# SharperJBCA/COMAPreduce

Measured on AMD Instinct MI355X. Metric: TOD samples x channels / s (L1 -> L2 reduction), higher is better.
Workload: dtype f32 in, f64 accumulate

## Files before the change

comapreduce_amd/csrc/l1_kernels.hip:

```cpp
#include "comap_internal.h"

#include <algorithm>
#include <cfloat>
#include <cmath>
#include <cstdlib>
#include <cstring>
#include <type_traits>
#include <utility>

using namespace comap;

#ifndef COMAP_GROUPS
#define COMAP_GROUPS 0
#endif
constexpr int kGroupsAutoMin = 3;

typedef float f32x4u __attribute__((ext_vector_type(4), aligned(4)));
__device__ __forceinline__ f32x4u ld4(const float *p)
{
    return __builtin_nontemporal_load(reinterpret_cast<const f32x4u *>(p));
}

__device__ __forceinline__ double wave_sum(double v)
{
// ... 911 lines not shown
                __double_as_longlong(kap[UC + i]) != __double_as_longlong(krfa) ||
                __double_as_longlong(kap[2 * UC + i]) != __double_as_longlong(kofa))
                atomicOr(flag, 1);
        }
        kap[i] = kgfa;
        kap[UC + i] = krfa;
        kap[2 * UC + i] = kofa;
        s_kap[0][c] = al;
        s_kap[1][c] = kgfa;
        s_kap[2][c] = krfa;
        s_kap[3][c] = kofa;
        if (fused) {
            const double sd = mom[i] - n * o - a * SA;
            if (kgfa != 0.0) { acc[0] += kgfa * o; acc[1] += kgfa * a; acc[2] += kgfa * sd; }
            if (krfa != 0.0) { acc[3] += krfa * o; acc[4] += krfa * a; acc[5] += krfa * sd; }
            if (kofa != 0.0) { acc[6] += kofa * o; acc[7] += kofa * a; acc[8] += kofa * sd; }
            if (kr != 0.0) acc[9] += kr;
        } else {
            if (kg != 0.0) { acc[0] += kg * fb; acc[1] += kg * fg; acc[2] += kg * fd; }
            if (kr != 0.0) { acc[3] += kr * fb; acc[4] += kr * fg; acc[5] += kr * fd; acc[9] += kr; }
            if (ko != 0.0) { acc[6] += ko * fb; acc[7] += ko * fg; acc[8] += ko * fd; }
        }
        acc[10] += W;
        acc[11] += Wo;
    }
#pragma unroll
    for (int k = 0; k < 12; ++k) acc[k] = block_sum256(acc[k], red);
    if (threadIdx.x == 0 && phase != 0) {
        if (fused) {
            const double *P = pd + 4 * (int64_t)ub;
#pragma unroll
            for (int j = 0; j < 3; ++j) {
                const double sko = acc[3 * j], ska = acc[3 * j + 1], ksy = acc[3 * j + 2];
                const double ksym = P[j] - Smf * sko - SAm * ska;
                const double kx0 = (Smm * ksy - Smf * ksym) / det;
                const double kx1 = (n * ksym - Smf * ksy) / det;
                acc[3 * j] = -(sko + kx0);
                acc[3 * j + 1] = -ska;
                acc[3 * j + 2] = -kx1;
            }
        }
        double *o = dsum + 16 * (int64_t)ub;
#pragma unroll
        for (int k = 0; k < 12; ++k) o[k] = acc[k];
    }
    if (phase == 0) {
        pbad = block_sum256(pbad, red);
        pmag = block_sum256(pmag, red);
        if (threadIdx.x == 0) {
            pg[2 * (int64_t)ub] = pbad;
            pg[2 * (int64_t)ub + 1] = pmag + 1.0;
        }
    }
    __syncthreads();
    if (phase == 0 && threadIdx.x < 64) {
        double *w = dw + 4 * (int64_t)ub * kChannels;
        const int nc = wave_compact_channels(
            threadIdx.x, [&](int c) { return s_kap[0][c] != 0.0; },
            [&](int j, int c) {
#pragma unroll
                for (int k = 0; k < 4; ++k) w[4 * j + k] = s_kap[k][c];
            },
            [&](int j) {
#pragma unroll
                for (int k = 0; k < 4; ++k) w[4 * j + k] = 0.0;
            },
            dlist + (int64_t)ub * kChannels);
        if (threadIdx.x == 0) dcnt[ub] = nc;
    }
}

__global__ void __launch_bounds__(256) k_special_rows(int mode, const int32_t *__restrict__ units,
                                                      const float *__restrict__ tod, int64_t T,
                                                      const double *__restrict__ A, const double *__restrict__ mf,
                                                      const double *__restrict__ oa, const double *__restrict__ alpha,
                                                      const double *__restrict__ nf, const int32_t *__restrict__ rowbad,
                                                      const double *__restrict__ bsum, const double *__restrict__ xreg,
                                                      const double *__restrict__ tsys0, const double *__restrict__ gain0,
                                                      const double *__restrict__ dsum, int calibrator,
                                                      int32_t *__restrict__ ugate, double *__restrict__ tod_out,
                                                      double *__restrict__ orig_out)
{
    __shared__ int nrow;
    __shared__ int16_t rows[kChannels];
    __shared__ double rw[kChannels], rwo[kChannels];
    const int ub = blockIdx.x;
    const int u = ub / kBands, b = ub % kBands;
    if (mode == 0 && b != 0) return;
    const int f = units[4 * u], t0 = units[4 * u + 2], n = units[4 * u + 3];
    const bool band_on = bsum[4 * (int64_t)ub + 3] > 0;
    if (!band_on) return;
    const bool zero = mode == 1 && !calibrator && n >= 5 && !ugate[u];
    if (threadIdx.x == 0) nrow = 0;
    __syncthreads();
    const int64_t kb = (int64_t)u * kBC + b * kChannels, fb = (int64_t)f * kBC + b * kChannels;
    for (int c = threadIdx.x; c < kChannels; c += blockDim.x) {
        const int64_t i = kb + c;
        if (!special_row(band_on, c, alpha[i], rowbad[i])) continue;
        const double tsv = tsys0[fb + c];
        if (zero && (gain_masked(c) || isnan(tsv))) continue;
        const float d0 = tod[(fb + c) * T + t0];
        const double y0 = special_y(alpha[i], oa[2 * i], oa[2 * i + 1], xreg[2 * i], xreg[2 * i + 1], d0,
                                    A[(int64_t)f * T + t0], mf[((int64_t)f * kBands + b) * T + t0]);
        double W, Wo;
        special_weights(c, tsv, nf[i], gain0[fb + c], y0, W, Wo);
        const int k = atomicAdd(&nrow, 1);
        rows[k] = (int16_t)c;
        rw[k] = W;
        rwo[k] = Wo;
    }
    __syncthreads();
    const int nr = nrow;
    if (nr == 0) return;
    const double *a = A + (int64_t)f * T + t0;
    const double *m = mf + ((int64_t)f * kBands + b) * T + t0;
    if (mode == 0) {
        bool inf = false;
        for (int t = threadIdx.x; t < n; t += blockDim.x)
            for (int k = 0; k < nr; ++k) {
                const int64_t i = kb + rows[k];
                const double y = special_y(alpha[i], oa[2 * i], oa[2 * i + 1], xreg[2 * i], xreg[2 * i + 1],
                                           tod[(fb + rows[k]) * T + t0 + t], a[t], m[t]);
                inf |= isinf(y);
            }
        if (inf) ugate[u] = 1;
        return;
    }
    const double *ds = dsum + 16 * (int64_t)ub;
    const double SW = ds[10], SWo = ds[11];
    double *to = tod_out + ((int64_t)f * kBands + b) * T + t0;
    double *oo = orig_out + ((int64_t)f * kBands + b) * T + t0;
    for (int t = threadIdx.x; t < n; t += blockDim.x) {
        double sr = 0.0, so = 0.0;
        for (int k = 0; k < nr; ++k) {
            const int c = rows[k];
            const int64_t i = kb + c;
            const double y = special_y(alpha[i], oa[2 * i], oa[2 * i + 1], xreg[2 * i], xreg[2 * i + 1],
                                       tod[(fb + c) * T + t0 + t], a[t], m[t]);
            double r = y * nf[i] / gain0[fb + c];
            if (isnan(r)) r = 0.0;
            sr += rw[k] * r;
            double q = y * tsys0[fb + c];
            if (isnan(q)) q = 0.0;
            so += rwo[k] * q;
        }
        to[t] += sr / SW;
        oo[t] += so / SWo;
    }
}

__global__ void __launch_bounds__(256) k_gain_avg(const float *__restrict__ tod, const double *__restrict__ A,
                                                  const int32_t *__restrict__ units, const int32_t *__restrict__ tiles,
                                                  int64_t tile0, int64_t T, int64_t UC, const double *__restrict__ kap,
                                                  const double *__restrict__ dsum, const double *__restrict__ mf,
                                                  double *__restrict__ tod_out, double *__restrict__ orig_out,
                                                  double *__restrict__ dG_out, const int32_t *__restrict__ flag)
{
    __shared__ double sg[kBands][kTile];
    if (*flag == 0) return;
    const int b = uniform(threadIdx.x >> 6);
    const int lane = threadIdx.x & 63;
    const int64_t tile = tile0 + blockIdx.x;
    const int u = tiles[2 * tile], toff = tiles[2 * tile + 1];
    const int f = units[4 * u], t0 = units[4 * u + 2], n = units[4 * u + 3];
    const int r0 = toff + 4 * lane;
    const float *base = tod + (int64_t)(f * kBands + b) * kChannels * T + t0 + r0;
    const int64_t kb = (int64_t)u * kBC + b * kChannels;
    const double *kg = kap + kb, *kr = kap + UC + kb, *ko = kap + 2 * UC + kb;
    double ag[4 * kJ], ar[4 * kJ], ao[4 * kJ];
#pragma unroll
    for (int i = 0; i < 4 * kJ; ++i) ag[i] = ar[i] = ao[i] = 0.0;
    const int nv0 = n - r0;
#pragma unroll 2
    for (int c = 0; c < kChannels; ++c) {
        const double wg = kg[c], wr = kr[c], wo = ko[c];
        if (wg == 0.0 && wr == 0.0 && wo == 0.0) continue;
        double x[4 * kJ];
        load_groups(base + (int64_t)c * T, nv0, x);
#pragma unroll
        for (int i = 0; i < 4 * kJ; ++i) {
            ag[i] = fma(wg, x[i], ag[i]);
            ar[i] = fma(wr, x[i], ar[i]);
            ao[i] = fma(wo, x[i], ao[i]);
        }
    }
    const double *ds = dsum + 16 * ((int64_t)u * kBands + b);
    const double *a = A + (int64_t)f * T + t0 + r0;
    const double *m = mf + (int64_t)(f * kBands + b) * T + t0 + r0;
    double at[4 * kJ], mt[4 * kJ];
#pragma unroll
    for (int g = 0; g < kJ; ++g)
#pragma unroll
        for (int e = 0; e < 4; ++e) {
            const int i = 4 * g + e, o = 256 * g + e;
            const bool ok = o < nv0;
            at[i] = ok ? a[o] : 0.0;
            mt[i] = ok ? m[o] : 0.0;
            sg[b][256 * g + 4 * lane + e] = ag[i] + ds[0] + at[i] * ds[1] + mt[i] * ds[2];
        }
    __syncthreads();
    double *to = tod_out + (int64_t)(f * kBands + b) * T + t0 + r0;
    double *oo = orig_out + (int64_t)(f * kBands + b) * T + t0 + r0;
#pragma unroll
    for (int g = 0; g < kJ; ++g)
#pragma unroll
        for (int e = 0; e < 4; ++e) {
            const int i = 4 * g + e, o = 256 * g + e;
            if (o >= nv0) continue;
            const int tl = 256 * g + 4 * lane + e;
            const double dG = sg[0][tl] + sg[1][tl] + sg[2][tl] + sg[3][tl];
            const double sr = ar[i] + ds[3] + at[i] * ds[4] + mt[i] * ds[5];
            const double so = ao[i] + ds[6] + at[i] * ds[7] + mt[i] * ds[8];
            to[o] = (sr - dG * ds[9]) / ds[10];
            oo[o] = so / ds[11];
            if (b == 0) dG_out[(int64_t)f * T + t0 + r0 + o] = dG;
        }
}

__device__ __forceinline__ void scan_weight_band(const double *__restrict__ r, int n, double *__restrict__ wo,
                                                 double *red)
{
    const int np = n / 2;
    double s = 0, cnt = 0;
    for (int k = threadIdx.x; k < np; k += blockDim.x) {
        const double d = r[2 * k + 1] - r[2 * k];
        if (!isnan(d)) { s += d; cnt += 1.0; }
    }
    s = block_sum256(s, red);
    cnt = block_sum256(cnt, red);
    const double mean = s / cnt;
    double v = 0;
    for (int k = threadIdx.x; k < np; k += blockDim.x) {
        const double d = r[2 * k + 1] - r[2 * k];
        if (!isnan(d)) v += (d - mean) * (d - mean);
    }
    v = block_sum256(v, red);
    const double rms = sqrt(v / cnt) / sqrt(2.0);
    const double wt = 1.0 / (rms * rms);
    for (int t = threadIdx.x; t < n; t += blockDim.x) wo[t] = wt;
}

__global__ void __launch_bounds__(256) k_scan_weights(int ub0, const int32_t *__restrict__ units, int64_t T,
                                                      const double *__restrict__ tod_out, double *__restrict__ w_out)
{
    __shared__ double red[4];
    const int ub = ub0 + blockIdx.x;
    const int u = ub / kBands, b = ub % kBands;
    const int f = units[4 * u], t0 = units[4 * u + 2], n = units[4 * u + 3];
    const int64_t o = (int64_t)(f * kBands + b) * T + t0;
    scan_weight_band(tod_out + o, n, w_out + o, red);
}

__global__ void __launch_bounds__(256) k_finish(const int32_t *__restrict__ units, const int32_t *__restrict__ tiles,
                                                int64_t tile0, int64_t T, const double *__restrict__ A,
                                                const double *__restrict__ mf, const double *__restrict__ dsum,
                                                double *__restrict__ tod_out, double *__restrict__ orig_out,
                                                double *__restrict__ dG, const int32_t *__restrict__ flag)
{
    if (*flag != 0) return;
    const int64_t tile = tile0 + blockIdx.x;
    const int u = tiles[2 * tile];
    const int f = units[4 * u], t0 = units[4 * u + 2], n = units[4 * u + 3];
    const double *ds = dsum + 16 * (int64_t)u * kBands;
    for (int k = threadIdx.x; k < kTile; k += 256) {
        const int r = tiles[2 * tile + 1] + k;
        if (r >= n) break;
        const int64_t t = t0 + r;
        const double a = A[(int64_t)f * T + t];
        double m[kBands], g = dG[(int64_t)f * T + t];
#pragma unroll
        for (int b = 0; b < kBands; ++b) {
            m[b] = mf[(int64_t)(f * kBands + b) * T + t];
            const double *d = ds + 16 * b;
            g += d[0] + a * d[1] + m[b] * d[2];
        }
        dG[(int64_t)f * T + t] = g;
#pragma unroll
        for (int b = 0; b < kBands; ++b) {
            const double *d = ds + 16 * b;
            const int64_t o = (int64_t)(f * kBands + b) * T + t;
            tod_out[o] = (tod_out[o] + d[3] + a * d[4] + m[b] * d[5] - g * d[9]) / d[10];
            orig_out[o] = (orig_out[o] + d[6] + a * d[7] + m[b] * d[8]) / d[11];
        }
    }
}

__global__ void __launch_bounds__(256) k_zero_gaps(const int64_t *__restrict__ gaps, int64_t T, int F,
                                                   double *__restrict__ tod_out, double *__restrict__ orig_out,
                                                   double *__restrict__ w_out)
{
    const int64_t *g = gaps + 3 * (int64_t)blockIdx.y;
    const int64_t f = g[0], t0 = g[1], n = g[2];
    for (int64_t k = blockIdx.x * (int64_t)blockDim.x + threadIdx.x; k < n; k += (int64_t)gridDim.x * blockDim.x) {
#pragma unroll
        for (int b = 0; b < kBands; ++b) {
            const int64_t o = (f * kBands + b) * T + t0 + k;
            tod_out[o] = 0.0;
            orig_out[o] = 0.0;
            w_out[o] = 0.0;
        }
    }
}

__global__ void __launch_bounds__(256) k_vane(const float *__restrict__ tod, int64_t T, int F,
                                              int64_t vstart, const int32_t *__restrict__ hot,
                                              const int64_t *__restrict__ hoff, const int32_t *__restrict__ cold,
                                              const int64_t *__restrict__ coff, double t_hot,
                                              double *__restrict__ tsys, double *__restrict__ gain)
{
    __shared__ float s_cold[128];
    const int side = threadIdx.x >> 7;
    const int64_t row = (int64_t)blockIdx.x * 128 + (threadIdx.x & 127);
    const bool live = row < (int64_t)F * kBC;
    const int fb = live ? (int)(row / kChannels) : 0;
    const float *p = tod + row * T + vstart;
    const int64_t h0 = hoff[fb], h1 = hoff[fb + 1], k0 = coff[fb], k1 = coff[fb + 1];
    float mean = 0.f;
    if (live && h1 != h0) {
        const int32_t *idx = side == 0 ? hot : cold;
        const int64_t j0 = side == 0 ? h0 : k0, j1 = side == 0 ? h1 : k1;
        float s = 0.f;
        int64_t cnt = 0;
        constexpr int kV = 16;
        int64_t j = j0;
        for (; j + kV <= j1; j += kV) {
            float x[kV];
#pragma unroll
            for (int k = 0; k < kV; ++k) x[k] = p[idx[j + k]];
#pragma unroll
            for (int k = 0; k < kV; ++k) {
                const bool ok = !isnan(x[k]);
                s += ok ? x[k] : 0.f;
                cnt += ok;
            }
        }
        for (; j < j1; ++j) {
            const float x = p[idx[j]];
            const bool ok = !isnan(x);
            s += ok ? x : 0.f;
            cnt += ok;
        }
        mean = (float)((double)s / (double)cnt);
    }
    if (side == 1) s_cold[threadIdx.x & 127] = mean;
    __syncthreads();
    if (side == 1 || !live) return;
    if (h1 == h0) {
        gain[row] = 0.0;
        tsys[row] = 0.0;
        return;
    }
    const float mc = s_cold[threadIdx.x];
    const float d = mean - mc;
    const double g = (double)d / (t_hot - 2.73);
    gain[row] = g;
    tsys[row] = (double)mc / g;
}

__global__ void __launch_bounds__(256) k_channel_bin(const float *__restrict__ tod, int64_t T, int32_t bw,
                                                     int32_t nbin, const double *__restrict__ w,
                                                     const double *__restrict__ g, const double *__restrict__ wsum,
                                                     double *__restrict__ avg, double *__restrict__ sd)
{
#pragma clang fp contract(off)
    const int b = uniform(threadIdx.x >> 6);
    const int lane = threadIdx.x & 63;
    const int64_t ntile = (T + kTile - 1) / kTile;
    const int f = (int)(blockIdx.x / ntile);
    const int64_t t0 = (int64_t)(blockIdx.x % ntile) * kTile;
    const int64_t r0 = t0 + 4 * lane;
    const int nv0 = (int)std::max<int64_t>(-1, std::min<int64_t>(T - r0, 1 << 20));
    const int64_t fb = (int64_t)f * kBands + b;
    const float *base = tod + fb * kChannels * T + r0;
    const double *wc = w + fb * kChannels, *gc = g + fb * kChannels;
    const bool full = t0 + kTile <= T;
    for (int k = 0; k < nbin; ++k) {
        double s1[4 * kJ], s2[4 * kJ];
#pragma unroll
        for (int i = 0; i < 4 * kJ; ++i) s1[i] = s2[i] = 0.0;
        for (int c = k * bw; c < (k + 1) * bw; ++c) {
            const double wv = wc[c], gv = gc[c];
            f32x4u r[kJ];
            if (full) load_raw<kJ, true>(base + (int64_t)c * T, nv0, r);
            else load_raw<kJ, false>(base + (int64_t)c * T, nv0, r);
#pragma unroll
            for (int q = 0; q < kJ; ++q)
#pragma unroll
                for (int e = 0; e < 4; ++e) {
                    const float x = (float)((double)r[q][e] / gv);
                    s1[4 * q + e] += (double)x * wv;
                    s2[4 * q + e] += (double)(x * x) * wv;
                }
        }
        const double W = wsum[fb * nbin + k];
        double *ao = avg + (fb * nbin + k) * T + r0, *so = sd + (fb * nbin + k) * T + r0;
#pragma unroll
        for (int q = 0; q < kJ; ++q)
#pragma unroll
            for (int e = 0; e < 4; ++e) {
                const int o = 256 * q + e;
                if (o >= nv0) continue;
                const double a = s1[4 * q + e] / W, sq = s2[4 * q + e] / W;
                ao[o] = a;
                so[o] = sqrt(sq - a * a);
            }
    }
}

static int prof_begin(comap_l1_plan *p, int id, hipStream_t st)
{
    if (!p->prof_on) return -1;
    if (p->prof_level == 1 && id != KV_MOMENTS && id != KV_BAND_SUMS && id != KV_REGRESS) return -1;
    const int idx = (int)p->prof_rec.size() * 2;
    while ((int)p->prof_pool.size() < idx + 2) {
        hipEvent_t e;
        if (hipEventCreate(&e) != hipSuccess) return -1;
        p->prof_pool.push_back(e);
    }
    (void)hipEventRecord(p->prof_pool[idx], st);
    return idx;
}

static void prof_end(comap_l1_plan *p, int id, int idx, hipStream_t st)
{
    if (idx < 0) return;
    (void)hipEventRecord(p->prof_pool[idx + 1], st);
    p->prof_rec.push_back({id, idx});
}

#define PROF_ON(p, id, st, ...)              \
    do {                                     \
        const int _pi = prof_begin(p, id, st); \
        __VA_ARGS__;                         \
        prof_end(p, id, _pi, st);            \
    } while (0)
#define PROF(p, id, ...) PROF_ON(p, id, (p)->ctx->stream, __VA_ARGS__)

extern "C" int comap_l1_profile(comap_l1_plan *p, int32_t enable)
{
    if (!p) return -1;
    p->prof_on = enable != 0;
    p->prof_level = enable >= 2 ? 2 : 1;
    return 0;
}

extern "C" int comap_l1_profile_collect(comap_l1_plan *p, double *ms, int64_t *counts, int32_t n)
{
    if (!p || !ms || !counts) return -1;
    COMAP_DEVICE_GUARD(p->ctx);
    comap_ctx *ctx = p->ctx;
    COMAP_CHECK(ctx, hipStreamSynchronize(ctx->stream));
    for (auto &r : p->prof_rec) {
        float t = 0.f;
        COMAP_CHECK(ctx, hipEventElapsedTime(&t, p->prof_pool[r.second], p->prof_pool[r.second + 1]));
        p->prof_ms[r.first] += t;
        p->prof_n[r.first] += 1;
    }
    p->prof_rec.clear();
    for (int i = 0; i < n && i < 32; ++i) {
        ms[i] = p->prof_ms[i];
        counts[i] = p->prof_n[i];
        p->prof_ms[i] = 0;
        p->prof_n[i] = 0;
    }
    return 0;
}

static int upload(comap_ctx *ctx, void **dst, const void *src, size_t bytes)
{
    COMAP_CHECK(ctx, hipMalloc(dst, bytes ? bytes : 8));
    if (bytes) COMAP_CHECK(ctx, hipMemcpyAsync(*dst, src, bytes, hipMemcpyHostToDevice, ctx->stream));
    return 0;
}

template <typename T>
static int dalloc(comap_ctx *ctx, T **p, size_t count)
{
    COMAP_CHECK(ctx, hipMalloc((void **)p, sizeof(T) * (count ? count : 1)));
    return 0;
}

extern "C" int comap_l1_plan_create(comap_ctx *ctx, const comap_obs_desc *d, comap_l1_plan **out)
{
    if (!ctx || !d || !out) return -1;
    COMAP_DEVICE_GUARD(ctx);
    if (d->n_bands != kBands || d->n_channels != kChannels)
        return comap_fail(ctx, -1, "only 4 bands x 1024 channels are supported");
    if (d->n_units <= 0 || d->n_samples <= 0 || d->n_feeds <= 0)
        return comap_fail(ctx, -1, "empty observation");
    COMAP_CHECK(ctx, hipSetDevice(ctx->device));
    auto *p = new comap_l1_plan();
    p->ctx = ctx;
    p->F = d->n_feeds; p->S = d->n_scans; p->U = d->n_units; p->T = d->n_samples;
    p->tod = d->tod; p->el = d->el;
    p->units_h.assign(d->units_host, d->units_host + 4 * (size_t)d->n_units);
    for (int u = 0; u < p->U; ++u) {
        const int32_t *q = &p->units_h[4 * u];
        if (q[0] < 0 || q[0] >= p->F || q[1] < 0 || q[1] >= p->S || q[2] < 0 || q[3] < 1 ||
            (int64_t)q[2] + q[3] > p->T) {
            delete p;
            return comap_fail(ctx, -1, "unit out of range");
        }
    }
    std::vector<int32_t> tiles;
    for (int u = 0; u < p->U; ++u)
        for (int t = 0; t < p->units_h[4 * u + 3]; t += kTile) { tiles.push_back(u); tiles.push_back(t); }
    p->n_tiles = (int64_t)tiles.size() / 2;
    std::vector<int32_t> tiles_b;
    std::vector<int64_t> tub(p->U + 1, 0);
    for (int u = 0; u < p->U; ++u) {
        const int shift = (p->T % 32 == 0) ? (p->units_h[4 * u + 2] & 31) : 0;
        for (int t = -shift; t < p->units_h[4 * u + 3]; t += kTile) { tiles_b.push_back(u); tiles_b.push_back(t); }
        tub[u + 1] = (int64_t)tiles_b.size() / 2;
    }
    std::vector<int64_t> gaps;
    {
        std::vector<std::vector<std::pair<int64_t, int64_t>>> cov(p->F);
        for (int u = 0; u < p->U; ++u)
            cov[p->units_h[4 * u]].push_back({p->units_h[4 * u + 2], p->units_h[4 * u + 2] + p->units_h[4 * u + 3]});
        for (int f = 0; f < p->F; ++f) {
            std::sort(cov[f].begin(), cov[f].end());
            int64_t t = 0;
            for (auto &c : cov[f]) {
                if (c.first > t) { gaps.push_back(f); gaps.push_back(t); gaps.push_back(c.first - t); }
                t = std::max(t, c.second);
            }
            if (t < p->T) { gaps.push_back(f); gaps.push_back(t); gaps.push_back(p->T - t); }
        }
        p->n_gaps = (int64_t)gaps.size() / 3;
        for (int64_t g = 0; g < p->n_gaps; ++g) p->max_gap = std::max(p->max_gap, gaps[3 * g + 2]);
    }
    const int64_t UC = (int64_t)p->U * kBC;
    int rc = 0;
    if (p->n_gaps) rc |= upload(ctx, (void **)&p->gaps, gaps.data(), gaps.size() * 8);
    rc |= dalloc(ctx, &p->flag, comap_l1_plan::kMaxGroups);
    rc |= dalloc(ctx, &p->dlist, (size_t)p->U * kBC);
    rc |= dalloc(ctx, &p->dcnt, (size_t)p->U * kBands);
    rc |= dalloc(ctx, &p->dw, 4 * (size_t)p->U * kBC);
    if (hipHostMalloc((void **)&p->nan_host, 4, hipHostMallocDefault) != hipSuccess) rc |= 1;
    if (hipEventCreateWithFlags(&p->mom_event, hipEventDisableTiming) != hipSuccess) rc |= 1;
    rc |= upload(ctx, (void **)&p->units, p->units_h.data(), p->units_h.size() * 4);
    rc |= upload(ctx, (void **)&p->tiles, tiles.data(), tiles.size() * 4);
    rc |= upload(ctx, (void **)&p->tiles_b, tiles_b.data(), tiles_b.size() * 4);
    rc |= dalloc(ctx, &p->airmass, (size_t)p->F * p->T);
    rc |= dalloc(ctx, &p->unit_sums, 8 * (size_t)p->U);
    rc |= dalloc(ctx, &p->mom, 5 * (size_t)UC);
    rc |= dalloc(ctx, &p->nan_count, 1);
    rc |= dalloc(ctx, &p->alpha, UC);
    rc |= dalloc(ctx, &p->nf, UC);
    rc |= dalloc(ctx, &p->bsum, 4 * (size_t)p->U * kBands);
    rc |= dalloc(ctx, &p->mb, (size_t)p->F * kBands * p->T);
    rc |= dalloc(ctx, &p->mf, (size_t)p->F * kBands * p->T);
    rc |= dalloc(ctx, &p->ssum, 4 * (size_t)p->U * kBands);
    rc |= dalloc(ctx, &p->sdm, UC);
    rc |= dalloc(ctx, &p->sgb, (size_t)p->F * kBands * p->T);
    rc |= dalloc(ctx, &p->pdot, 4 * (size_t)p->U * kBands);
    rc |= dalloc(ctx, &p->pgate, 2 * (size_t)p->U * kBands);
    rc |= dalloc(ctx, &p->needc, (size_t)p->U * kBands);
    rc |= dalloc(ctx, &p->gw, (size_t)p->F * kBC);
    rc |= dalloc(ctx, &p->gmode, p->F);
    rc |= dalloc(ctx, &p->kap, 3 * (size_t)UC);
    rc |= dalloc(ctx, &p->dsum, 16 * (size_t)p->U * kBands);
    rc |= dalloc(ctx, &p->xreg, 2 * (size_t)UC);
    rc |= dalloc(ctx, &p->dG, (size_t)p->F * p->T);
    rc |= dalloc(ctx, &p->rowbad, UC);
    rc |= dalloc(ctx, &p->ubs, 4 * (size_t)p->U * kBands);
    rc |= dalloc(ctx, &p->fitsum, 2 * (size_t)UC);
    rc |= dalloc(ctx, &p->oa, 2 * (size_t)UC);
    rc |= dalloc(ctx, &p->ynf, (size_t)p->U);
    rc |= dalloc(ctx, &p->ugate, (size_t)p->U);
    if (rc) { delete p; return -2; }
    if (const char *r = getenv("COMAP_L1_REGRESS")) {
        if (!strcmp(r, "legacy")) p->regress_legacy = true;
        else if (strcmp(r, "fused")) { comap_l1_plan_destroy(p); return comap_fail(ctx, -1, "COMAP_L1_REGRESS must be fused or legacy"); }
    }
    int groups = COMAP_GROUPS;
    if (groups <= 0) {
        int per_cu = 0, cus = 0;
        if (hipOccupancyMaxActiveBlocksPerMultiprocessor(&per_cu, k_band_sums, 256, 0) != hipSuccess) per_cu = 0;
        if (hipDeviceGetAttribute(&cus, hipDeviceAttributeMultiprocessorCount, ctx->device) != hipSuccess) cus = 0;
        const int64_t resident = (int64_t)per_cu * cus, fill = resident * 7 / 8, blocks = (int64_t)kSubB * tub[p->U];
        groups = fill > 0 ? (int)std::min<int64_t>(comap_l1_plan::kMaxGroups, (blocks + fill - 1) / fill) : 1;
        if (groups < kGroupsAutoMin || blocks * 10 < groups * resident * 7) groups = 1;
    }
    if (const char *g = getenv("COMAP_GROUPS")) groups = atoi(g);
    p->ngroups = std::max(1, std::min(std::min(groups, comap_l1_plan::kMaxGroups), (int)p->U));
    if (const char *r = getenv("COMAP_L1_PIPE")) {
        if (!strcmp(r, "alt")) p->pipe_alt = true;
        else if (strcmp(r, "chain")) { comap_l1_plan_destroy(p); return comap_fail(ctx, -1, "COMAP_L1_PIPE must be chain or alt"); }
    }
    {
        std::vector<int64_t> tu(p->U + 1, 0);
        for (int u = 0; u < p->U; ++u) tu[u + 1] = tu[u] + (p->units_h[4 * u + 3] + kTile - 1) / kTile;
        for (int g = 0; g <= p->ngroups; ++g) {
            p->grp_u0[g] = (int32_t)((int64_t)p->U * g / p->ngroups);
            p->grp_tile0[g] = tu[p->grp_u0[g]];
            p->grpb_tile0[g] = tub[p->grp_u0[g]];
        }
    }
    int prio = 0;
    if (const char *sp = getenv("COMAP_SIDE_PRIO"); sp && sp[0] == '1') {
        int lo = 0, hi = 0;
        if (hipDeviceGetStreamPriorityRange(&lo, &hi) == hipSuccess) prio = hi;
    }
    bool ok = hipStreamCreateWithPriority(&p->side, hipStreamNonBlocking, prio) == hipSuccess;
    for (int g = 0; g < p->ngroups && ok; ++g)
        ok = hipEventCreateWithFlags(&p->ev_b[g], hipEventDisableTiming) == hipSuccess &&
             hipEventCreateWithFlags(&p->ev_m[g], hipEventDisableTiming) == hipSuccess;
    ok = ok && hipEventCreateWithFlags(&p->ev_pre, hipEventDisableTiming) == hipSuccess &&
         hipEventCreateWithFlags(&p->ev_join, hipEventDisableTiming) == hipSuccess;
    if (!ok) { comap_l1_plan_destroy(p); return comap_fail(ctx, -2, "side stream / events"); }
    for (int g = 0; g < p->ngroups; ++g) {
        std::vector<MedJob> jobs;
        for (int u = p->grp_u0[g]; u < p->grp_u0[g + 1]; ++u) {
            const int32_t f = p->units_h[4 * u], t0 = p->units_h[4 * u + 2], n = p->units_h[4 * u + 3];
            for (int b = 0; b < kBands; ++b) {
                MedJob j;
                const int64_t off = (int64_t)(f * kBands + b) * p->T + t0;
                j.src = p->mb + off;
                j.dst = p->mf + off;
                j.n = n;
                j.out_lo = n;
                j.out_hi = (n >= 2 * kMedfiltWindow) ? 2 * (int64_t)n : (int64_t)n;
                j.mode = 1;
                j.pad_ = 0;
                j.gate = p->bsum + 4 * ((int64_t)u * kBands + b) + 3;
                jobs.push_back(j);
            }
        }
        rc = comap_median_plan(ctx, &p->medg[g], jobs, kMedfiltWindow);
        if (rc) { comap_l1_plan_destroy(p); return rc; }
    }
    k_airmass<<<2048, 256, 0, ctx->stream>>>(p->el, p->airmass, (int64_t)p->F * p->T);
    COMAP_LAUNCH_CHECK(ctx);
    k_unit_sums<<<p->U, 256, 0, ctx->stream>>>(p->units, p->airmass, p->T, p->unit_sums);
    COMAP_LAUNCH_CHECK(ctx);
    *out = p;
    return 0;
}

extern "C" int comap_l1_plan_destroy(comap_l1_plan *p)
{
    if (!p) return 0;
    COMAP_DEVICE_GUARD(p->ctx);
    if (p->side) (void)hipStreamSynchronize(p->side);
    void *bufs[] = {p->units, p->tiles, p->tiles_b, p->gaps, p->airmass, p->unit_sums, p->mom,
                    p->nan_count, p->alpha, p->nf, p->bsum, p->mb, p->mf, p->ssum, p->sdm, p->gw,
                    p->gmode, p->kap, p->dsum, p->xreg, p->dG, p->rowbad, p->ubs, p->fitsum, p->oa,
                    p->flag, p->dlist, p->dcnt, p->dw, p->nanpos, p->nanpos_n, p->vane_dev,
                    p->sel_pairs, p->sel_voff, p->sel_flag, p->sel_valid, p->ynf, p->ugate, p->sgb, p->pdot,
                    p->pgate, p->needc};
    for (void *b : bufs)
        if (b) (void)hipFree(b);
    for (int g = 0; g < comap_l1_plan::kMaxGroups; ++g) {
        comap_median_plan_free(&p->medg[g]);
// ... 496 lines not shown
```

Before: 769.0 billion.

## Restructure vane calibration gather to coalesce columns via LDS transpose

```diff
diff --git a/comapreduce_amd/csrc/l1_kernels.hip b/comapreduce_amd/csrc/l1_kernels.hip
--- a/comapreduce_amd/csrc/l1_kernels.hip
+++ b/comapreduce_amd/csrc/l1_kernels.hip
@@ -1237,55 +1237,59 @@
     }
 }
 
+constexpr int kVR = 32, kVC = 32;
 __global__ void __launch_bounds__(256) k_vane(const float *__restrict__ tod, int64_t T, int F,
                                               int64_t vstart, const int32_t *__restrict__ hot,
                                               const int64_t *__restrict__ hoff, const int32_t *__restrict__ cold,
                                               const int64_t *__restrict__ coff, double t_hot,
                                               double *__restrict__ tsys, double *__restrict__ gain)
 {
-    __shared__ float s_cold[128];
-    const int side = threadIdx.x >> 7;
-    const int64_t row = (int64_t)blockIdx.x * 128 + (threadIdx.x & 127);
-    const bool live = row < (int64_t)F * kBC;
-    const int fb = live ? (int)(row / kChannels) : 0;
-    const float *p = tod + row * T + vstart;
-    const int64_t h0 = hoff[fb], h1 = hoff[fb + 1], k0 = coff[fb], k1 = coff[fb + 1];
-    float mean = 0.f;
-    if (live && h1 != h0) {
-        const int32_t *idx = side == 0 ? hot : cold;
-        const int64_t j0 = side == 0 ? h0 : k0, j1 = side == 0 ? h1 : k1;
-        float s = 0.f;
-        int64_t cnt = 0;
-        constexpr int kV = 16;
-        int64_t j = j0;
-        for (; j + kV <= j1; j += kV) {
-            float x[kV];
-#pragma unroll
-            for (int k = 0; k < kV; ++k) x[k] = p[idx[j + k]];
-#pragma unroll
-            for (int k = 0; k < kV; ++k) {
-                const bool ok = !isnan(x[k]);
-                s += ok ? x[k] : 0.f;
+    __shared__ float tile[4][2 * kVR * (kVC + 1)];
+    const int wid = uniform(threadIdx.x >> 6), lane = threadIdx.x & 63;
+    const int64_t row0 = (int64_t)blockIdx.x * 128 + wid * kVR;
+    if (row0 >= (int64_t)F * kBC) return;
+    const int fb = (int)(row0 / kChannels);
+    const int64_t h0 = hoff[fb], k0 = coff[fb];
+    const int nh = (int)(hoff[fb + 1] - h0), nc = (int)(coff[fb + 1] - k0);
+    const int gs = lane >> 5, ge = lane & 31, ss = lane & 1;
+    const int32_t *gidx = gs ? cold + k0 : hot + h0;
+    const int gn = gs ? nc : nh, sn = ss ? nc : nh;
+    const float *p = tod + row0 * T + vstart;
+    float *buf = tile[wid];
+    float s = 0.f;
+    int64_t cnt = 0;
+    if (nh != 0) {
+        const int nmax = nh > nc ? nh : nc;
+        for (int j0 = 0; j0 < nmax; j0 += kVC) {
+            const int64_t col = j0 + ge < gn ? gidx[j0 + ge] : 0;
+            float x[kVR];
+#pragma unroll
+            for (int r = 0; r < kVR; ++r) x[r] = p[r * T + col];
+#pragma unroll
+            for (int r = 0; r < kVR; ++r) buf[(2 * r + gs) * (kVC + 1) + ge] = x[r];
+            __builtin_amdgcn_fence(__ATOMIC_ACQ_REL, "wavefront");
+            __builtin_amdgcn_wave_barrier();
+            const float *q = buf + lane * (kVC + 1);
+            const int m = sn - j0 < kVC ? sn - j0 : kVC;
+            for (int k = 0; k < m; ++k) {
+                const float v = q[k];
+                const bool ok = !isnan(v);
+                s += ok ? v : 0.f;
                 cnt += ok;
             }
-        }
-        for (; j < j1; ++j) {
-            const float x = p[idx[j]];
-            const bool ok = !isnan(x);
-            s += ok ? x : 0.f;
-            cnt += ok;
-        }
-        mean = (float)((double)s / (double)cnt);
-    }
-    if (side == 1) s_cold[threadIdx.x & 127] = mean;
-    __syncthreads();
-    if (side == 1 || !live) return;
-    if (h1 == h0) {
+            __builtin_amdgcn_fence(__ATOMIC_ACQ_REL, "wavefront");
+            __builtin_amdgcn_wave_barrier();
+        }
+    }
+    const float mean = (float)((double)s / (double)cnt);
+    const float mc = __shfl_down(mean, 1, 64);
+    if (ss == 1) return;
+    const int64_t row = row0 + (lane >> 1);
+    if (nh == 0) {
         gain[row] = 0.0;
         tsys[row] = 0.0;
         return;
     }
-    const float mc = s_cold[threadIdx.x];
     const float d = mean - mc;
     const double g = (double)d / (t_hot - 2.73);
     gain[row] = g;
```

New measurement: 775.3 billion (median of 6 runs). No clear change (+0.8%).
